# jbikker/tinybvh

Measured on AMD Instinct MI355X. Metric: MRays/s (primary + diffuse) on Bistro CWBVH, higher is better.
Workload: dtype f32; 1 GPU; procedural street (Bistro-exterior stand-in, 2.83M tris, seed 2); BVH8_CWBVH; per GPU per step 16777216 primary + 16777216 diffuse (depth 1-3) Intersect; scene_tris=2832120, layout=BVH8_CWBVH, scene_is_stand_in=True

## Files before the change

include/tinybvh_amd_debug.h:

```cpp
#ifndef TINYBVH_AMD_DEBUG_H_
#define TINYBVH_AMD_DEBUG_H_
#include "tinybvh_amd.h"
#ifdef __cplusplus
extern "C" {
#endif

int tbvh_debug_stats(tbvh_context* ctx, uint64_t out[8], int reset);

int tbvh_debug_set_flags(tbvh_context* ctx, uint32_t flags);

int tbvh_debug_coherent_schedule(tbvh_scene* scene, int anyhit, uint32_t out[4]);

int tbvh_debug_last_probe(tbvh_context* ctx, uint32_t out[3]);

int tbvh_debug_overlap_stats(tbvh_context* ctx, uint64_t out[2]);
int tbvh_debug_lane_script(const uint64_t* ops5, uint64_t n_ops, int32_t* out);

int tbvh_set_variant(tbvh_scene* scene, int variant);

int tbvh_debug_wide_copy_bvh2(int layout, const void* blob, uint64_t n_blob, const uint32_t* prim_idx, uint64_t n_idx, const void* verts16, uint64_t n_tris,
                              uint32_t max_leaf_tris, void* nodes32_out, uint64_t cap_nodes, uint64_t* n_nodes_out, void* recs_out, uint64_t cap_recs,
                              uint64_t* n_recs_out);

int tbvh_debug_set_sah_small_subtree(tbvh_context* ctx, uint32_t n);

int tbvh_debug_device_allocations(uint64_t out[2]);

struct tbvh_scenegraph;
int tbvh_debug_scenegraph_array(struct tbvh_scenegraph* g, int what, void** d_ptr);
int tbvh_debug_scenegraph_step(struct tbvh_scenegraph* g, int step, float dt);
struct tbvh_host_scenegraph;
int tbvh_debug_host_scenegraph_set_trs(struct tbvh_host_scenegraph* g, const float* trs10, uint64_t n_nodes);
int tbvh_debug_host_scenegraph_check_chains(struct tbvh_host_scenegraph* g, uint64_t* n_differ);

#ifdef __cplusplus
}
#endif
#endif
```

tinybvh_amd/_capi.py:

```python
from __future__ import annotations

import ctypes as C
import os

_HERE = os.path.dirname(os.path.abspath(__file__))
LIB_PATH = os.environ.get("TBVH_LIB_OVERRIDE") or os.path.join(_HERE, "libtinybvh_amd.so")

_u64, _u32, _vp, _i = C.c_uint64, C.c_uint32, C.c_void_p, C.c_int
_pp = C.POINTER(C.c_void_p)


class BuildParams(C.Structure):
    _fields_ = [("bins", _u32), ("max_leaf_tris", _u32), ("threads", _u32), ("flags", _u32)]


class Mesh(C.Structure):
    _fields_ = [("verts", C.c_void_p), ("n_verts", C.c_uint64), ("stride_bytes", C.c_uint32), ("on_device", C.c_uint32),
                ("indices", C.c_void_p), ("n_tris", C.c_uint64)]


class AlphaTexture(C.Structure):
    _fields_ = [("texels", C.c_void_p), ("width", C.c_uint32), ("height", C.c_uint32)]


class OmmSource(C.Structure):
    _fields_ = [("uv", C.c_void_p), ("n_uv", C.c_uint64), ("uv_stride_bytes", C.c_uint32), ("on_device", C.c_uint32), ("indices", C.c_void_p),
                ("n_tris", C.c_uint64), ("tri_texture", C.c_void_p), ("textures", C.POINTER(AlphaTexture)), ("n_textures", C.c_uint32)]


class SceneGraphDesc(C.Structure):
    _fields_ = [("flags", C.c_uint32), ("n_nodes", C.c_uint64), ("parent", C.c_void_p), ("visit_order", C.c_void_p), ("translation", C.c_void_p), ("rotation", C.c_void_p),
                ("scale", C.c_void_p), ("matrix", C.c_void_p), ("local_transform", C.c_void_p), ("n_weights", C.c_void_p), ("weights", C.c_void_p),
                ("n_samplers", C.c_uint64), ("sampler_interpolation", C.c_void_p), ("sampler_type", C.c_void_p), ("sampler_key_offset", C.c_void_p),
                ("sampler_value_offset", C.c_void_p), ("key_times", C.c_void_p), ("key_values", C.c_void_p), ("n_animations", C.c_uint64), ("n_channels", C.c_uint64),
                ("channel_animation", C.c_void_p), ("channel_sampler", C.c_void_p), ("channel_node", C.c_void_p), ("channel_target", C.c_void_p),
                ("n_instances", C.c_uint64), ("node_of_instance", C.c_void_p), ("n_skin_uses", C.c_uint64), ("skin_mesh_node", C.c_void_p),
                ("skin_joint_offset", C.c_void_p), ("skin_joint_node", C.c_void_p), ("skin_inverse_bind", C.c_void_p)]


class Camera(C.Structure):
    _fields_ = [("eye", C.c_float * 3), ("p1", C.c_float * 3), ("p2", C.c_float * 3), ("p3", C.c_float * 3),
                ("width", _u32), ("height", _u32), ("spp_x", _u32), ("spp_y", _u32)]


class WfParams(C.Structure):
    _fields_ = [("light_pos", C.c_float * 3), ("light_color", C.c_float * 3), ("sky_lo", C.c_float * 3), ("sky_hi", C.c_float * 3),
                ("eps", C.c_float), ("max_depth", _u32), ("seed", _u32), ("clear", _u32), ("light_size", C.c_float * 2), ("flags", _u32), ("sample_index", _u32)]


class WfStats(C.Structure):
    _fields_ = [("extend_rays", _u64 * 8), ("shadow_rays", _u64 * 8), ("frame_ms", C.c_float)]


SYMBOLS = {
    "tbvh_debug_wide_copy_bvh2": (_i, [_i, _vp, _u64, _vp, _u64, _vp, _u64, _u32, _vp, _u64, C.POINTER(_u64), _vp, _u64, C.POINTER(_u64)]),
    "tbvh_wavefront_create": (_i, [_vp, _u32, _u32, _pp]),
    "tbvh_wavefront_destroy": (None, [_vp]),
    "tbvh_wavefront_render": (_i, [_vp, _vp, _vp, C.POINTER(Camera), C.POINTER(WfParams), C.POINTER(WfStats)]),
    "tbvh_wavefront_read": (_i, [_vp, _vp]),
    "tbvh_wavefront_set_blas_vertices": (_i, [_vp, _vp, _u64]),
    "tbvh_wavefront_finalize": (_i, [_vp, C.c_float, _vp]),
    "tbvh_wavefront_set_blue_noise": (_i, [_vp, _vp, _u64]),
    "tbvh_abi_version": (_i, []),
    "tbvh_last_error": (C.c_char_p, []),
    "tbvh_device_count": (_i, []),
    "tbvh_init": (_i, [_i, _pp]),
    "tbvh_shutdown": (None, [_vp]),
    "tbvh_synchronize": (_i, [_vp]),
    "tbvh_set_stream": (_i, [_vp, _vp]),
    "tbvh_context_set_overlap": (_i, [_vp, _i]),
    "tbvh_debug_overlap_stats": (_i, [_vp, _vp]),
    "tbvh_debug_lane_script": (_i, [_vp, _u64, _vp]),
    "tbvh_set_timing": (_i, [_vp, _i]),
    "tbvh_upload_bvh_gpu": (_i, [_vp, _vp, _u64, _vp, _u64, _vp, _u64, _pp]),
    "tbvh_upload_bvh4_gpu": (_i, [_vp, _vp, _u64, _pp]),
    "tbvh_upload_cwbvh": (_i, [_vp, _vp, _u64, _vp, _u64, _pp]),
    "tbvh_upload_tlas": (_i, [_vp, _vp, _u64, _vp, _u64, _vp, _u64, _pp, _u64, _pp]),
    "tbvh_update_tlas": (_i, [_vp, _vp, _u64, _vp, _u64, _vp, _u64]),
    "tbvh_update_bvh_gpu": (_i, [_vp, _vp, _u64, _vp, _u64, _vp, _u64]),
    "tbvh_update_bvh4_gpu": (_i, [_vp, _vp, _u64]),
    "tbvh_update_cwbvh": (_i, [_vp, _vp, _u64, _vp, _u64]),
    "tbvh_rebuild_tlas_device": (_i, [_vp, _vp, _i, _vp, _u64]),
    "tbvh_refit": (_i, [_vp, _vp, _u64, _i]),
    "tbvh_set_opacity_micromaps": (_i, [_vp, _vp, _u32, _u64, _i]),
    "tbvh_scene_download": (_i, [_vp, _i, _vp, _u64, _vp]),
    "tbvh_build_device": (_i, [_vp, _vp, _u64, _i, _i, _u32, _vp]),
    "tbvh_build_device_ploc": (_i, [_vp, _vp, _u64, _i, _i, _u32, _vp]),
    "tbvh_build_device_sah": (_i, [_vp, _vp, _u64, _i, _i, _u32, _vp]),
    "tbvh_build_bvh2_sah_device": (_i, [_vp, C.POINTER(Mesh), _u32, _vp, _u64, _vp, _u64, _i, C.POINTER(_u64)]),
    "tbvh_host_build_bvh2_sah": (_i, [C.POINTER(Mesh), _u32, _vp, _u64, _vp, _u64, C.POINTER(_u64)]),
    "tbvh_convert_bvh2_device": (_i, [_vp, _vp, _u64, _vp, _u64, _vp, _u64, _i, _i, _vp]),
    "tbvh_tlas_download": (_i, [_vp, _vp, _u64, _vp, _u64, _vp, _u64, _vp]),
    "tbvh_free_scene": (None, [_vp]),
    "tbvh_scene_layout": (_i, [_vp]),
    "tbvh_scene_device_bytes": (_u64, [_vp]),
    "tbvh_intersect": (_i, [_vp, _vp, _u64, _u32]),
    "tbvh_occluded": (_i, [_vp, _vp, _u64, _u32, _vp]),
    "tbvh_intersect_sharded": (_i, [_vp, _u32, _vp, _u64, _u32]),
    "tbvh_occluded_sharded": (_i, [_vp, _u32, _vp, _u64, _u32, _vp]),
    "tbvh_intersect_sharded_device": (_i, [_vp, _u32, _vp, _vp, _i, C.c_float, _vp, _vp]),
    "tbvh_occluded_sharded_device": (_i, [_vp, _u32, _vp, _vp, _vp, _vp, _vp]),
    "tbvh_wavefront_set_band": (_i, [_vp, _u32, _u32]),
    "tbvh_wavefront_render_sharded": (_i, [_vp, _vp, _vp, _u32, C.POINTER(Camera), _vp, _vp, _vp]),
    "tbvh_wavefront_read_sharded": (_i, [_vp, _u32, _vp]),
    "tbvh_shard_range": (None, [_u64, _u32, _u32, C.POINTER(_u64), C.POINTER(_u64)]),
    "tbvh_intersect_device": (_i, [_vp, _vp, _u64]),
    "tbvh_occluded_device": (_i, [_vp, _vp, _u64, _vp]),
    "tbvh_intersect_device_fresh": (_i, [_vp, _vp, _u64, C.c_float]),
    "tbvh_reset_hits_device": (_i, [_vp, _vp, _u64, C.c_float]),
    "tbvh_time_last_ms": (C.c_float, [_vp]),
    "tbvh_debug_coherent_schedule": (C.c_int, [_vp, C.c_int, C.POINTER(C.c_uint32)]),
    "tbvh_time_history": (C.c_int, [_vp, C.POINTER(C.c_float), C.c_uint32, C.POINTER(C.c_uint32)]),
    "tbvh_measure_copy_bandwidth": (_i, [_vp, _u64, _u32, C.POINTER(C.c_double)]),
    "tbvh_measure_read_bandwidth": (_i, [_vp, _u64, _u32, C.POINTER(C.c_double)]),
    "tbvh_measure_valu_issue": (_i, [_vp, _u32, C.POINTER(C.c_double)]),
    "tbvh_measure_link_bandwidth": (_i, [_vp, _u64, _u32, C.POINTER(C.c_double), C.POINTER(C.c_double)]),
    "tbvh_scene_get_schedule_hint": (_i, [_vp, _vp]),
    "tbvh_scene_set_schedule_hint": (_i, [_vp, _vp]),
    "tbvh_pinned_malloc": (_i, [_vp, _u64, _pp]),
    "tbvh_pinned_free": (_i, [_vp, _vp]),
    "tbvh_set_variant": (_i, [_vp, _i]),
    "tbvh_debug_stats": (_i, [_vp, _vp, _i]),
    "tbvh_debug_last_probe": (_i, [_vp, _vp]),
    "tbvh_debug_set_flags": (_i, [_vp, _u32]),
    "tbvh_debug_set_sah_small_subtree": (_i, [_vp, _u32]),
    "tbvh_debug_device_allocations": (_i, [C.POINTER(_u64)]),
    "tbvh_cwbvh_set_hybrid": (_i, [_vp, C.c_int64]),
    "tbvh_bin_rays_device": (_i, [_vp, _vp, _vp, _u64, C.POINTER(C.c_float), _u32, _u32, _vp]),
    "tbvh_generate_primary_device": (_i, [_vp, C.POINTER(Camera), _vp, _u64, _u64]),
    "tbvh_generate_bounce_device": (_i, [_vp, _vp, _vp, _vp, _u64, _u32]),
    "tbvh_generate_shadow_device": (_i, [_vp, _vp, _vp, _u64, C.POINTER(C.c_float), C.c_float]),
    "tbvh_device_malloc": (_i, [_vp, _u64, _pp]),
    "tbvh_device_free": (_i, [_vp, _vp]),
    "tbvh_copy_to_device": (_i, [_vp, _vp, _vp, _u64]),
    "tbvh_copy_from_device": (_i, [_vp, _vp, _vp, _u64]),
    "tbvh_host_build": (_i, [_vp, _u64, _i, C.POINTER(BuildParams), _pp]),
    "tbvh_host_build_tlas": (_i, [_vp, _u64, _vp, _u64, _pp]),
    "tbvh_host_free": (None, [_vp]),
    "tbvh_cwbvh_file_write": (_i, [C.c_char_p, _vp, _u64, _vp, _u64, _u64, _vp]),
    "tbvh_cwbvh_file_read": (_i, [C.c_char_p, _u64, _pp, C.POINTER(_u64)]),
    "tbvh_host_layout": (_i, [_vp]),
    "tbvh_host_blob": (_vp, [_vp, _i]),
    "tbvh_host_blob_count": (_u64, [_vp, _i]),
    "tbvh_upload_host": (_i, [_vp, _vp, _vp, _u64, _pp]),
    "tbvh_upload_bvh_double": (_i, [_vp, _vp, _u64, _vp, _u64, _vp, _u64, _pp]),
    "tbvh_upload_tlas_double": (_i, [_vp, _vp, _u64, _vp, _u64, _vp, _u64, _pp, _u64, _pp]),
    "tbvh_intersect_ex_device": (_i, [_vp, _vp, _u64]),
    "tbvh_occluded_ex_device": (_i, [_vp, _vp, _u64, _vp]),
    "tbvh_intersect_ex": (_i, [_vp, _vp, _u64]),
    "tbvh_occluded_ex": (_i, [_vp, _vp, _u64, _vp]),
    "tbvh_host_build_double": (_i, [_vp, _u64, _pp]),
    "tbvh_host_build_tlas_double": (_i, [_vp, _u64, _vp, _u64, _pp]),
    "tbvh_rebuild_tlas_double_device": (_i, [_vp, _vp, _i]),
    "tbvh_update_tlas_double": (_i, [_vp, _vp, _u64, _vp, _u64, _vp, _u64]),
    "tbvh_tlas_double_download": (_i, [_vp, _vp, _u64, _vp, _u64, _vp, _u64, _vp]),
# ... 109 lines not shown
```

tinybvh_amd/csrc/capi_context.hip:

```cpp
#include "capi_internal.h"

using namespace tbvh;
using namespace tbvh_capi;

namespace {
thread_local char g_err[512] = "";
}

namespace tbvh_capi {
int fail(int code, const char* fmt, ...) {
    va_list ap;
    va_start(ap, fmt);
    vsnprintf(g_err, sizeof g_err, fmt, ap);
    va_end(ap);
    return code;
}

int joinLanes(tbvh_context* c) {
    if (c->lane1Dirty) {
        HIP_TRY(hipStreamWaitEvent(c->stream, c->lane1Last, 0));
        c->lane1Dirty = false;
        c->laneJoins++;
    }
    c->book.joined();
    c->lane0Touched = true;
    c->chain++;
    if (!c->chain) c->chain = 1;
    return 0;
}
int setDevice(tbvh_context* c) {
    HIP_TRY(hipSetDevice(c->device));
    return joinLanes(c);
}
hipError_t timedBegin(tbvh_context* c, hipStream_t lane) {
    if (c->skipTiming) return hipSuccess;
    const uint32_t slot = (uint32_t)(c->evSeq % tbvh_context::kTimeRing);
    for (int k = 0; k < 2; k++)
        if (!c->evRing[slot][k]) { const hipError_t e = hipEventCreate(&c->evRing[slot][k]); if (e != hipSuccess) return e; }
    c->evDone[slot] = false;
    c->evChain[slot] = 0;
    c->ev0 = c->evRing[slot][0]; c->ev1 = c->evRing[slot][1];
    c->evSeq++;
    return hipEventRecord(c->ev0, lane ? lane : c->stream);
}
hipError_t timedEnd(tbvh_context* c, hipStream_t lane) {
    if (c->skipTiming) return hipSuccess;
    const hipError_t e = hipEventRecord(c->ev1, lane ? lane : c->stream);
    if (e == hipSuccess && c->evSeq) { c->evDone[(c->evSeq - 1) % tbvh_context::kTimeRing] = true; c->timed = true; }
    return e;
}
float timedMs(tbvh_context* c, uint64_t seq) {
    constexpr uint64_t R = tbvh_context::kTimeRing;
    const uint32_t slot = (uint32_t)(seq % R);
    float own = -1.0f;
    if (hipEventElapsedTime(&own, c->evRing[slot][0], c->evRing[slot][1]) != hipSuccess) { (void)hipGetLastError(); return -1.0f; }
    const uint32_t chain = c->evChain[slot];
    if (!chain) return own;
    constexpr uint64_t kReach = 2 * LaneBook::kMaxInFlight;
    const uint64_t oldest = c->evSeq > R ? c->evSeq - R : 0;
    const uint64_t lo = seq > oldest + kReach ? seq - kReach : oldest, hi = seq + kReach < c->evSeq ? seq + kReach + 1 : c->evSeq;
    float from = 0.f;
    for (uint64_t j = lo; j < hi; j++) {
        const uint32_t sj = (uint32_t)(j % R);
        if (j == seq || c->evChain[sj] != chain || !c->evDone[sj]) continue;
        float endJ = 0.f;
        if (hipEventSynchronize(c->evRing[sj][1]) != hipSuccess || hipEventElapsedTime(&endJ, c->evRing[slot][0], c->evRing[sj][1]) != hipSuccess) { (void)hipGetLastError(); continue; }
        const bool before = endJ < own || (endJ == own && j < seq);
        if (before && endJ > from) from = endJ;
    }
    return own - from;
}
}

extern "C" {

int tbvh_abi_version(void) { return TBVH_ABI_VERSION; }
const char* tbvh_last_error(void) { return g_err; }

int tbvh_device_count(void) {
    int n = 0;
    hipError_t e = hipGetDeviceCount(&n);
    if (e != hipSuccess) { fail(TBVH_E_HIP, "hipGetDeviceCount: %s", hipGetErrorString(e)); return e == hipErrorNoDevice ? 0 : TBVH_E_HIP; }
    return n;
// ... 56 lines not shown
    if (c->lane1.stream) hipStreamSynchronize(c->lane1.stream);
    if (c->ownStream) hipStreamSynchronize(c->ownStream);
    c->lane1Dirty = false;
    for (;;) {
        tbvh_scene* t = nullptr;
        for (tbvh_scene* s : c->scenes) if (s->isTlas) { t = s; break; }
        if (!t) break;
        tbvh_free_scene(t);
    }
    while (!c->scenes.empty()) tbvh_free_scene(c->scenes.back());
    freePosesOf(c);
    freeGraphsOf(c);
    freeShadingsOf(c);
    freeOmmStagingOf(c);
    for (const tbvh_context::PinnedRange& r : c->pinned) hipHostFree(r.host);
    c->pinned.clear();
    delete c->pipe;
    for (auto& pair : c->evRing) for (hipEvent_t ev : pair) if (ev) hipEventDestroy(ev);
    if (c->evBase) hipEventDestroy(c->evBase);
    if (c->lane1.stream) hipStreamDestroy(c->lane1.stream);
    if (c->ownStream) hipStreamDestroy(c->ownStream);
    delete c;
}

int tbvh_debug_device_allocations(uint64_t out[2]) {
    if (!out) return fail(TBVH_E_INVALID, "tbvh_debug_device_allocations: null argument");
    out[0] = g_devBufLive.load(); out[1] = g_devBufBytes.load();
    return 0;
}

int tbvh_synchronize(tbvh_context* c) {
    if (!c) return fail(TBVH_E_INVALID, "null context");
    TBVH_ENTER(c);
    HIP_TRY(hipStreamSynchronize(c->stream));
    return 0;
}

int tbvh_set_stream(tbvh_context* c, void* s) {
    if (!c) return fail(TBVH_E_INVALID, "null context");
    TBVH_ENTER(c);
    c->stream = s ? (hipStream_t)s : c->ownStream;
    return 0;
}

int tbvh_context_set_overlap(tbvh_context* c, int enabled) {
    if (!c) return fail(TBVH_E_INVALID, "tbvh_context_set_overlap: null context");
    TBVH_ENTER(c);
    c->overlap = enabled != 0;
    return 0;
}

int tbvh_debug_lane_script(const uint64_t* ops5, uint64_t nOps, int32_t* out) {
    if ((!ops5 || !out) && nOps) return fail(TBVH_E_INVALID, "tbvh_debug_lane_script: null argument");
    LaneBook book;
    std::vector<uint8_t> done(nOps, 0);
    bool allowLane1 = true;
    auto prune = [&] { book.prune([&](int, uint32_t slot) { return done[slot] != 0; }); };
    for (uint64_t i = 0; i < nOps; i++) {
        const uint64_t* op = ops5 + i * 5;
        out[i] = 0;
        switch (op[0]) {
        case 0: {
            LaneFootprint fp;
            fp.rays.lo = (uintptr_t)op[1]; fp.rays.hi = (uintptr_t)op[2]; fp.occ.lo = (uintptr_t)op[3]; fp.occ.hi = (uintptr_t)op[4];
            prune();
            const LaneChoice ch = book.decide(fp, allowLane1);
            if (ch.join) book.joined();
            book.add(ch.lane, fp, (uint32_t)i);
            out[i] = ch.lane + (ch.join ? 2 : 0);
            break;
        }
        case 1:
            if (op[1] >= nOps) return fail(TBVH_E_INVALID, "tbvh_debug_lane_script: row %llu finishes a row beyond the script", (unsigned long long)i);
            done[op[1]] = 1;
            break;
        case 2: allowLane1 = op[1] != 0; break;
        case 3: prune(); out[i] = book.count[0] + 256 * book.count[1]; break;
        default: return fail(TBVH_E_INVALID, "tbvh_debug_lane_script: row %llu has no such operation", (unsigned long long)i);
        }
    }
    return 0;
}

int tbvh_debug_overlap_stats(tbvh_context* c, uint64_t out[2]) {
    if (!c || !out) return fail(TBVH_E_INVALID, "tbvh_debug_overlap_stats: null argument");
    TBVH_LOCK(c);
    out[0] = c->lane1Launches; out[1] = c->laneJoins;
    return 0;
}

float tbvh_time_last_ms(tbvh_context* c) {
    if (!c) return -1.0f;
    TBVH_LOCK(c);
    if (!c->timed) return -1.0f;
    if (c->hostQuerySeq == c->evSeq && c->hostQueryMs >= 0.f) return c->hostQueryMs;
    hipSetDevice(c->device);
    if (hipEventSynchronize(c->ev1) != hipSuccess) return -1.0f;
    if (c->evSeq && c->ev1 == c->evRing[(c->evSeq - 1) % tbvh_context::kTimeRing][1]) return timedMs(c, c->evSeq - 1);
    float ms = -1.0f;
    if (hipEventElapsedTime(&ms, c->ev0, c->ev1) != hipSuccess) return -1.0f;
    return ms;
}

int tbvh_time_history(tbvh_context* c, float* ms, uint32_t cap, uint32_t* count) {
    if (!c || !count || (!ms && cap)) return fail(TBVH_E_INVALID, "tbvh_time_history: null argument");
    *count = 0;
    TBVH_ENTER(c);
    uint64_t n = c->evSeq < tbvh_context::kTimeRing ? c->evSeq : tbvh_context::kTimeRing;
    if (n > cap) n = cap;
    for (uint64_t i = 0; i < n; i++) {
        const uint32_t slot = (uint32_t)((c->evSeq - n + i) % tbvh_context::kTimeRing);
        float t = -1.0f;
        if (c->evDone[slot]) {
            HIP_TRY(hipEventSynchronize(c->evRing[slot][1]));
            t = timedMs(c, c->evSeq - n + i);
            if (t < 0.f && !c->evChain[slot]) HIP_TRY(hipEventElapsedTime(&t, c->evRing[slot][0], c->evRing[slot][1]));
        }
        ms[i] = t;
    }
    *count = (uint32_t)n;
    return 0;
}

int tbvh_debug_stats(tbvh_context* c, uint64_t out[8], int reset) {
    if (!c || !out) return fail(TBVH_E_INVALID, "tbvh_debug_stats: null argument");
    TBVH_ENTER(c);
    HIP_TRY(hipStreamSynchronize(c->stream));
    HIP_TRY(hipMemcpy(out, c->counter + 8, 64, hipMemcpyDeviceToHost));
    if (reset) HIP_TRY(hipMemset(c->counter + 8, 0, 64));
    return 0;
}

int tbvh_set_timing(tbvh_context* c, int enabled) {
    if (!c) return fail(TBVH_E_INVALID, "tbvh_set_timing: null context");
    TBVH_LOCK(c);
    c->skipTiming = enabled == 0;
    return 0;
}

int tbvh_debug_set_flags(tbvh_context* c, uint32_t flags) {
    if (!c) return fail(TBVH_E_INVALID, "tbvh_debug_set_flags: null context");
    TBVH_LOCK(c);
    c->expFlags = flags;
    return 0;
}

int tbvh_debug_last_probe(tbvh_context* c, uint32_t out[3]) {
    if (!c || !out) return fail(TBVH_E_INVALID, "tbvh_debug_last_probe: null argument");
    TBVH_ENTER(c);
    out[0] = out[1] = out[2] = 0;
    if (!c->lastProbed) return 0;
    HIP_TRY(hipStreamSynchronize(c->stream));
    const uint32_t* pool = c->lastProbedLane ? c->lane1.pool.get() : c->pool.get();
    const int last = (c->lastProbedLane ? c->lane1.poolCur : c->poolCur) ^ 1;
    HIP_TRY(hipMemcpy(out, pool + (size_t)last * ((size_t)(kPoolParts + 1) * kPoolCounterStride) + (size_t)kPoolParts * kPoolCounterStride, 8, hipMemcpyDeviceToHost));
    out[2] = (out[1] != 0 && out[0] * 10u >= out[1] * 6u) ? 2u : 1u;
    return 0;
}


int tbvh_device_malloc(tbvh_context* c, uint64_t bytes, void** out) {
    if (!c || !out) return fail(TBVH_E_INVALID, "tbvh_device_malloc: null argument");
    TBVH_ENTER(c);
    hipError_t e = hipMalloc(out, bytes ? bytes : 16);
    if (e != hipSuccess) return fail(TBVH_E_NOMEM, "hipMalloc(%llu): %s", (unsigned long long)bytes, hipGetErrorString(e));
    return 0;
// ... 108 lines not shown
```

tinybvh_amd/csrc/cwbvh_packet.h:

```cpp
#pragma once
#include "device_common.h"
#include "cwbvh_node.h"

namespace tbvh {

constexpr int kPacketWG = 64;

__device__ __forceinline__ uint32_t sgpr(uint32_t v) { return (uint32_t)__builtin_amdgcn_readfirstlane((int)v); }

template <bool MIXED>
__device__ __forceinline__ uint32_t pk_test_children(const float (*planes)[8], float ax, float ay, float az, float ox, float oy, float oz, float tcull,
                                                     uint32_t m0, uint32_t m1, uint32_t oct0) {
    const uint32_t lane = threadIdx.x;
    const uint32_t metaL = ((lane & 4u) ? m1 : m0) >> (8u * (lane & 3u)) & 255u;
    const bool innerL = (metaL & 0x18u) == 0x18u;
    const uint32_t placedL = (metaL >> 5) << ((innerL ? (metaL ^ oct0) : metaL) & 31u);
    const uint32_t nonEmpty = (uint32_t)wave_ballot(lane < 8u && metaL != 0u);
    uint32_t hitmask = 0;
    float4 pa = *(const float4*)&planes[0][0];
    float2 pb = *(const float2*)&planes[0][4];
#pragma unroll
    for (int c = 0; c < 8; c++) {
        const float4 qa = pa; const float2 qb = pb;
        if (c < 7) { pa = *(const float4*)&planes[c + 1][0]; pb = *(const float2*)&planes[c + 1][4]; }
        if (!((nonEmpty >> c) & 1u)) continue;
        float tnx = __builtin_fmaf(qa.x, ax, ox), tny = __builtin_fmaf(qa.y, ay, oy), tnz = __builtin_fmaf(qa.z, az, oz);
        float tfx = __builtin_fmaf(qa.w, ax, ox), tfy = __builtin_fmaf(qb.x, ay, oy), tfz = __builtin_fmaf(qb.y, az, oz);
        if (MIXED) {
            const float a0 = __builtin_fminf(tnx, tfx), a1 = __builtin_fmaxf(tnx, tfx), b0 = __builtin_fminf(tny, tfy), b1 = __builtin_fmaxf(tny, tfy);
            const float c0 = __builtin_fminf(tnz, tfz), c1 = __builtin_fmaxf(tnz, tfz);
            tnx = a0; tfx = a1; tny = b0; tfy = b1; tnz = c0; tfz = c1;
        }
        const float cmin = __builtin_fmaxf(cw_fmax3(tnx, tny, tnz), 0.0f);
        const float cmax = __builtin_fminf(cw_fmin3(tfx, tfy, tfz), tcull);
        const uint32_t placed = (uint32_t)__builtin_amdgcn_readlane((int)placedL, c);
        hitmask |= wave_ballot(cmin <= cmax) != 0ull ? placed : 0u;
    }
    return hitmask;
}

}
```

tinybvh_amd/csrc/kernels_cwbvh_packet.hip:

```cpp
#include "device_common.h"
#include "ray_pool.h"
#include "kernels.h"
#include "cwbvh_node.h"
#include "cwbvh_probe.h"
#include "cwbvh_packet.h"

namespace tbvh {

namespace {

constexpr int WG = 64;

template <bool ANYHIT, bool HAS_OMM>
__global__ __launch_bounds__(WG, 8) void k_cwbvh_packet(const float4* __restrict__ nodes, const float4* __restrict__ tris, QueryArgs q, uint32_t* __restrict__ status) {
    __shared__ float planes[8][8];
    const uint64_t nRaysTotal = q.nRaysDev ? *q.nRaysDev : q.nRays;
    RayPool<64> pool;
    pool.init(q.poolParts, q.counterNext);
    if (q.probe) {
        uint32_t agree, pairs;
        coherence_sample(q.rays, nRaysTotal, q.fresh != 0u, q.freshTmax, agree, pairs);
        if (blockIdx.x == 0 && threadIdx.x == 0) { q.probe[0] = agree; q.probe[1] = pairs; }
        if (!((pairs != 0 && agree * 10u >= pairs * 6u) || (q.flags & 16u) != 0)) return;
    }
    uint2* const spill = (uint2*)q.spill + (size_t)blockIdx.x * WG;
    const size_t spillRow = (size_t)gridDim.x * WG;
    const uint32_t spillCap = q.spillStride * (uint32_t)WG;
    bool overflow = false;
    const uint32_t lane = threadIdx.x;

    for (;;) {
        uint64_t ri = 0;
        const bool have = pool.acquire(true, q.counter, nRaysTotal, ri);
        if (wave_ballot(have) == 0) break;
        float3 O = make_float3(0, 0, 0), D = make_float3(0, 0, 1), rD = make_float3(1e30f, 1e30f, 1);
        float4 hit = make_float4(0, 0, 0, 0);
        if (have) {
            const RayRec* rp = q.rays + ri;
            O = xyz(rp->O); D = xyz(rp->D); rD = xyz(rp->rD);
            hit = q.fresh ? make_float4(q.freshTmax, 0.f, 0.f, 0.f) : rp->hit;
        }
        bool found = false;
        bool on = have;
        const uint32_t oct = 7u - ((rD.x < 0 ? 4u : 0u) | (rD.y < 0 ? 2u : 0u) | (rD.z < 0 ? 1u : 0u));
        const unsigned long long haveMask = wave_ballot(have);
        const uint32_t first = (uint32_t)__builtin_ctzll(haveMask);
        const uint32_t oct0 = (uint32_t)__builtin_amdgcn_readlane((int)oct, (int)first);
        const bool mixed = wave_ballot(have && oct != oct0) != 0;
        const bool negX0 = ((7u - oct0) & 4u) != 0, negY0 = ((7u - oct0) & 2u) != 0, negZ0 = ((7u - oct0) & 1u) != 0;
        const uint32_t p = lane >> 3, axis = p % 3u, isHi = p / 3u;
        const bool negA = axis == 0 ? negX0 : axis == 1 ? negY0 : negZ0;
        const uint32_t dstPlane = axis + 3u * (isHi ^ (negA ? 1u : 0u));
        float* const myPlane = &planes[lane & 7u][lane < 48u ? dstPlane : 6u + ((lane >> 3) & 1u)];

        uint32_t sp = 0;
        uint32_t ngx = 0, ngy = 0x80000000u;
        uint32_t stkx = 0, stky = 0;
        auto pick = [&](uint32_t& ci) -> bool {
            if (!(ngy > 0x00FFFFFFu)) {
                if (sp == 0) return false;
                sp--;
                if (sp < 64u) { ngx = (uint32_t)__builtin_amdgcn_readlane((int)stkx, (int)sp); ngy = (uint32_t)__builtin_amdgcn_readlane((int)stky, (int)sp); }
                else { const uint32_t j_ = sp - 64u; const uint2 e = spill[(j_ & 63u) + (size_t)(j_ >> 6) * spillRow]; ngx = sgpr(e.x); ngy = sgpr(e.y); }
            }
            const uint32_t imaskWord = ngy;
            const uint32_t bit = 31u - (uint32_t)__builtin_clz(ngy);
            ngy &= ~(1u << bit);
            if (ngy > 0x00FFFFFFu) {
                if (sp < 64u) { const bool mine = lane == sp; stkx = mine ? ngx : stkx; stky = mine ? ngy : stky; }
                else {
                    const uint32_t j_ = sp - 64u;
                    if (j_ < spillCap) { if (lane == 0) spill[(j_ & 63u) + (size_t)(j_ >> 6) * spillRow] = make_uint2(ngx, ngy); }
                    else { overflow = true; sp--; }
                }
                sp++;
            }
            const uint32_t slot = (bit - 24u) ^ oct0;
            ci = sgpr(ngx + (uint32_t)__popc(imaskWord & ~(0xFFFFFFFFu << slot)));
            return true;
        };
        uint32_t ci = 0;
        bool more = pick(ci);
        float4 n0 = make_float4(0, 0, 0, 0), n1 = n0;
        uint32_t qb = 0;
        auto fetch = [&](uint32_t c_) {
            const float4* np = nodes + (size_t)c_ * 5u;
            n0 = np[0]; n1 = np[1];
            qb = ((const uint8_t*)(np + 2))[lane < 48u ? lane : 47u];
        };
        if (more) fetch(ci);
        while (more) {
            __builtin_amdgcn_wave_barrier();
            *myPlane = (float)qb;
            __builtin_amdgcn_wave_barrier();
            const uint32_t ew = sgpr(as_u32(n0.w));
            const float ax = ldexpf(rD.x, (int)(int8_t)(ew)), ay = ldexpf(rD.y, (int)(int8_t)(ew >> 8)), az = ldexpf(rD.z, (int)(int8_t)(ew >> 16));
            const float ox = (n0.x - O.x) * rD.x, oy = (n0.y - O.y) * rD.y, oz = (n0.z - O.z) * rD.z;
            const bool lives = ANYHIT ? (on && !found) : on;
            const float tcull = lives ? cull_bound(hit.x) : -1.0f;
            const uint32_t m0 = sgpr(as_u32(n1.z)), m1 = sgpr(as_u32(n1.w));
            const uint32_t hitmask = mixed ? pk_test_children<true>(planes, ax, ay, az, ox, oy, oz, tcull, m0, m1, oct0)
                                           : pk_test_children<false>(planes, ax, ay, az, ox, oy, oz, tcull, m0, m1, oct0);
            ngx = sgpr(as_u32(n1.x));
            ngy = (hitmask & 0xFF000000u) | (ew >> 24);
            uint32_t tgy = hitmask & 0x00FFFFFFu;
            const uint32_t tgx = sgpr(as_u32(n1.y));
            more = pick(ci);
            if (more) fetch(ci);
            while (tgy != 0u) {
                const uint32_t ti = 31u - (uint32_t)__builtin_clz(tgy);
                tgy &= ~(1u << ti);
                const float4* tp = tris + ((size_t)tgx + ti * 3u);
                const float4 e2 = tp[0], e1 = tp[1], v0 = tp[2];
                TriHit h;
                if ((ANYHIT ? (on && !found) : on) &&
                    tri_test(O, D, xyz(v0), xyz(e1), xyz(e2), hit.x, h, HAS_OMM ? q.omm : Omm{nullptr, 0}, as_u32(v0.w)) &&
                    (ANYHIT || hit_wins(h.t, as_u32(v0.w), found, hit))) {
                    found = true;
                    if (!ANYHIT) hit = make_float4(h.t, h.u, h.v, v0.w);
                }
            }
            if (ANYHIT && wave_ballot(on && !found) == 0ull) break;
        }
        if (have) {
            if (ANYHIT) q.occluded[ri] = found ? 1 : 0;
            else if (found || q.fresh) q.rays[ri].hit = hit;
        }
    }
    if (overflow) atomicOr(status, 1u);
}

}

void launch_cwbvh_packet(bool anyhit, const float4* nodes, const float4* tris, const QueryArgs& q, uint32_t* status, uint32_t blocks, hipStream_t s) {
    if (anyhit) {
        if (q.omm.map) hipLaunchKernelGGL((k_cwbvh_packet<true, true>), dim3(blocks), dim3(WG), 0, s, nodes, tris, q, status);
        else hipLaunchKernelGGL((k_cwbvh_packet<true, false>), dim3(blocks), dim3(WG), 0, s, nodes, tris, q, status);
    } else {
        if (q.omm.map) hipLaunchKernelGGL((k_cwbvh_packet<false, true>), dim3(blocks), dim3(WG), 0, s, nodes, tris, q, status);
        else hipLaunchKernelGGL((k_cwbvh_packet<false, false>), dim3(blocks), dim3(WG), 0, s, nodes, tris, q, status);
    }
}

}
```

Baseline: 5166 MRays/s.

## Add conservative packet-interval culling of CWBVH children before per-lane exact tests

For coherent, non-anyhit packets whose rays share one octant and are all finite, the kernel computes wave-wide min/max of origins and inverse directions plus the maximum cull distance. Each node's child boxes are then tested once against this interval bound, and only surviving children get the exact per-lane ballot test. The aim is to skip per-child FMA work and ballots for children no ray can hit. In exchange it adds wave reductions at packet start and after every hit update, more shared memory, and extra per-node plane math. It also adds a host debug entry point that reproduces the cull logic.

```diff
diff --git a/include/tinybvh_amd_debug.h b/include/tinybvh_amd_debug.h
--- a/include/tinybvh_amd_debug.h
+++ b/include/tinybvh_amd_debug.h
@@ -15,6 +15,9 @@
 
 int tbvh_debug_overlap_stats(tbvh_context* ctx, uint64_t out[2]);
 int tbvh_debug_lane_script(const uint64_t* ops5, uint64_t n_ops, int32_t* out);
+
+int tbvh_debug_packet_cull(const void* nodes80, uint64_t n_nodes, const void* rays64, uint64_t have_mask, const float* tcull64, uint8_t* maybe_out,
+                           uint8_t* exact_out, uint32_t* chunk_flags);
 
 int tbvh_set_variant(tbvh_scene* scene, int variant);
 
diff --git a/tinybvh_amd/_capi.py b/tinybvh_amd/_capi.py
--- a/tinybvh_amd/_capi.py
+++ b/tinybvh_amd/_capi.py
@@ -71,6 +71,7 @@
     "tbvh_context_set_overlap": (_i, [_vp, _i]),
     "tbvh_debug_overlap_stats": (_i, [_vp, _vp]),
     "tbvh_debug_lane_script": (_i, [_vp, _u64, _vp]),
+    "tbvh_debug_packet_cull": (_i, [_vp, _u64, _vp, _u64, _vp, _vp, _vp, _vp]),
     "tbvh_set_timing": (_i, [_vp, _i]),
     "tbvh_upload_bvh_gpu": (_i, [_vp, _vp, _u64, _vp, _u64, _vp, _u64, _pp]),
     "tbvh_upload_bvh4_gpu": (_i, [_vp, _vp, _u64, _pp]),
diff --git a/tinybvh_amd/csrc/capi_context.hip b/tinybvh_amd/csrc/capi_context.hip
--- a/tinybvh_amd/csrc/capi_context.hip
+++ b/tinybvh_amd/csrc/capi_context.hip
@@ -1,4 +1,5 @@
 #include "capi_internal.h"
+#include "packet_cull.h"
 
 using namespace tbvh;
 using namespace tbvh_capi;
@@ -221,6 +222,75 @@
     return 0;
 }
 
+int tbvh_debug_packet_cull(const void* nodes80, uint64_t nNodes, const void* rays64, uint64_t haveMask, const float* tcull64, uint8_t* maybeOut, uint8_t* exactOut,
+                           uint32_t* chunkFlags) {
+    if (!rays64 || !tcull64 || haveMask == 0 || (nNodes && (!nodes80 || !maybeOut || !exactOut)))
+        return fail(TBVH_E_INVALID, "tbvh_debug_packet_cull: null argument or no lane holds a ray");
+    using namespace tbvh;
+    float O[64][3], rD[64][3];
+    uint32_t oct[64];
+    for (int l = 0; l < 64; l++) {
+        const float* r = (const float*)((const uint8_t*)rays64 + 64 * l);
+        for (int a = 0; a < 3; a++) { O[l][a] = r[a]; rD[l][a] = r[8 + a]; }
+        oct[l] = 7u - ((rD[l][0] < 0 ? 4u : 0u) | (rD[l][1] < 0 ? 2u : 0u) | (rD[l][2] < 0 ? 1u : 0u));
+    }
+    const int first = __builtin_ctzll(haveMask);
+    const uint32_t oct0 = oct[first];
+    const bool neg0[3] = {((7u - oct0) & 4u) != 0, ((7u - oct0) & 2u) != 0, ((7u - oct0) & 1u) != 0};
+    bool mixed = false, raysFinite = true;
+    float Olo[3], Ohi[3], rlo[3], rhi[3], TC = -1.0f;
+    for (int a = 0; a < 3; a++) { Olo[a] = Ohi[a] = O[first][a]; rlo[a] = rhi[a] = rD[first][a]; }
+    for (int l = 0; l < 64; l++) {
+        if (!((haveMask >> l) & 1u)) continue;
+        mixed |= oct[l] != oct0;
+        for (int a = 0; a < 3; a++) {
+            raysFinite &= pkc_finite(O[l][a]) && pkc_finite(rD[l][a]);
+            Olo[a] = __builtin_fminf(Olo[a], O[l][a]); Ohi[a] = __builtin_fmaxf(Ohi[a], O[l][a]);
+            rlo[a] = __builtin_fminf(rlo[a], rD[l][a]); rhi[a] = __builtin_fmaxf(rhi[a], rD[l][a]);
+        }
+        TC = __builtin_fmaxf(TC, pk_cull_tc(tcull64[l]));
+    }
+    const bool useCull = !mixed && raysFinite;
+    if (chunkFlags) *chunkFlags = (mixed ? 1u : 0u) | (raysFinite ? 0u : 2u);
+    for (uint64_t n = 0; n < nNodes; n++) {
+        const uint8_t* node = (const uint8_t*)nodes80 + 80 * n;
+        float n0[3];
+        uint32_t ew;
+        memcpy(n0, node, 12); memcpy(&ew, node + 12, 4);
+        const int e[3] = {(int)(int8_t)ew, (int)(int8_t)(ew >> 8), (int)(int8_t)(ew >> 16)};
+        const uint8_t* meta = node + 24;
+        const uint8_t* qbytes = node + 32;
+        float planes[8][6], bounds[8][6];
+        bool allFinite = true;
+        for (uint32_t L = 0; L < 48; L++) {
+            const uint32_t p = L >> 3, axis = p % 3u, isHi = p / 3u, dstPlane = axis + 3u * (isHi ^ (neg0[axis] ? 1u : 0u));
+            const float qf = (float)qbytes[L];
+            planes[L & 7u][dstPlane] = qf;
+            bool fin;
+            bounds[L & 7u][dstPlane] = pk_cull_plane(dstPlane >= 3u, qf, n0[axis], e[axis], Olo[axis], Ohi[axis], rlo[axis], rhi[axis], fin);
+            allFinite &= fin;
+        }
+        float ax[64][3], ox[64][3];
+        for (int l = 0; l < 64; l++)
+            for (int a = 0; a < 3; a++) { ax[l][a] = ldexpf(rD[l][a], e[a]); ox[l][a] = (n0[a] - O[l][a]) * rD[l][a]; }
+        uint32_t maybe = 0, exact = 0;
+        for (uint32_t c = 0; c < 8; c++) {
+            if (meta[c] == 0) continue;
+            const float* b = bounds[c];
+            if (!useCull || pk_cull_pass(b[0], b[1], b[2], b[3], b[4], b[5], TC, allFinite)) maybe |= 1u << c;
+            const float* q = planes[c];
+            for (int l = 0; l < 64 && !((exact >> c) & 1u); l++) {
+                if (!((haveMask >> l) & 1u)) continue;
+                const bool in = mixed ? pk_child_exact<true>(q[0], q[1], q[2], q[3], q[4], q[5], ax[l][0], ax[l][1], ax[l][2], ox[l][0], ox[l][1], ox[l][2], tcull64[l])
+                                      : pk_child_exact<false>(q[0], q[1], q[2], q[3], q[4], q[5], ax[l][0], ax[l][1], ax[l][2], ox[l][0], ox[l][1], ox[l][2], tcull64[l]);
+                if (in) exact |= 1u << c;
+            }
+        }
+        maybeOut[n] = (uint8_t)maybe; exactOut[n] = (uint8_t)exact;
+    }
+    return 0;
+}
+
 int tbvh_debug_overlap_stats(tbvh_context* c, uint64_t out[2]) {
     if (!c || !out) return fail(TBVH_E_INVALID, "tbvh_debug_overlap_stats: null argument");
     TBVH_LOCK(c);
diff --git a/tinybvh_amd/csrc/cwbvh_packet.h b/tinybvh_amd/csrc/cwbvh_packet.h
--- a/tinybvh_amd/csrc/cwbvh_packet.h
+++ b/tinybvh_amd/csrc/cwbvh_packet.h
@@ -1,6 +1,7 @@
 #pragma once
 #include "device_common.h"
 #include "cwbvh_node.h"
+#include "packet_cull.h"
 
 namespace tbvh {
 
@@ -8,14 +9,20 @@
 
 __device__ __forceinline__ uint32_t sgpr(uint32_t v) { return (uint32_t)__builtin_amdgcn_readfirstlane((int)v); }
 
-template <bool MIXED>
-__device__ __forceinline__ uint32_t pk_test_children(const float (*planes)[8], float ax, float ay, float az, float ox, float oy, float oz, float tcull,
-                                                     uint32_t m0, uint32_t m1, uint32_t oct0) {
+struct PkMeta { uint32_t placedL, nonEmpty; };
+__device__ __forceinline__ PkMeta pk_meta(uint32_t m0, uint32_t m1, uint32_t oct0) {
     const uint32_t lane = threadIdx.x;
     const uint32_t metaL = ((lane & 4u) ? m1 : m0) >> (8u * (lane & 3u)) & 255u;
     const bool innerL = (metaL & 0x18u) == 0x18u;
-    const uint32_t placedL = (metaL >> 5) << ((innerL ? (metaL ^ oct0) : metaL) & 31u);
-    const uint32_t nonEmpty = (uint32_t)wave_ballot(lane < 8u && metaL != 0u);
+    PkMeta m;
+    m.placedL = (metaL >> 5) << ((innerL ? (metaL ^ oct0) : metaL) & 31u);
+    m.nonEmpty = (uint32_t)wave_ballot(metaL != 0u) & 0xFFu;
+    return m;
+}
+
+template <bool MIXED>
+__device__ __forceinline__ uint32_t pk_test_children_of(const float (*planes)[8], float ax, float ay, float az, float ox, float oy, float oz, float tcull,
+                                                        uint32_t placedL, uint32_t todo) {
     uint32_t hitmask = 0;
     float4 pa = *(const float4*)&planes[0][0];
     float2 pb = *(const float2*)&planes[0][4];
@@ -23,20 +30,43 @@
     for (int c = 0; c < 8; c++) {
         const float4 qa = pa; const float2 qb = pb;
         if (c < 7) { pa = *(const float4*)&planes[c + 1][0]; pb = *(const float2*)&planes[c + 1][4]; }
-        if (!((nonEmpty >> c) & 1u)) continue;
-        float tnx = __builtin_fmaf(qa.x, ax, ox), tny = __builtin_fmaf(qa.y, ay, oy), tnz = __builtin_fmaf(qa.z, az, oz);
-        float tfx = __builtin_fmaf(qa.w, ax, ox), tfy = __builtin_fmaf(qb.x, ay, oy), tfz = __builtin_fmaf(qb.y, az, oz);
-        if (MIXED) {
-            const float a0 = __builtin_fminf(tnx, tfx), a1 = __builtin_fmaxf(tnx, tfx), b0 = __builtin_fminf(tny, tfy), b1 = __builtin_fmaxf(tny, tfy);
-            const float c0 = __builtin_fminf(tnz, tfz), c1 = __builtin_fmaxf(tnz, tfz);
-            tnx = a0; tfx = a1; tny = b0; tfy = b1; tnz = c0; tfz = c1;
-        }
-        const float cmin = __builtin_fmaxf(cw_fmax3(tnx, tny, tnz), 0.0f);
-        const float cmax = __builtin_fminf(cw_fmin3(tfx, tfy, tfz), tcull);
+        if (!((todo >> c) & 1u)) continue;
         const uint32_t placed = (uint32_t)__builtin_amdgcn_readlane((int)placedL, c);
-        hitmask |= wave_ballot(cmin <= cmax) != 0ull ? placed : 0u;
+        hitmask |= wave_ballot(pk_child_exact<MIXED>(qa.x, qa.y, qa.z, qa.w, qb.x, qb.y, ax, ay, az, ox, oy, oz, tcull)) != 0ull ? placed : 0u;
     }
     return hitmask;
 }
 
+template <bool MIXED>
+__device__ __forceinline__ uint32_t pk_test_children(const float (*planes)[8], float ax, float ay, float az, float ox, float oy, float oz, float tcull,
+                                                     uint32_t m0, uint32_t m1, uint32_t oct0) {
+    const PkMeta m = pk_meta(m0, m1, oct0);
+    return pk_test_children_of<MIXED>(planes, ax, ay, az, ox, oy, oz, tcull, m.placedL, m.nonEmpty);
 }
+
+__device__ __forceinline__ uint32_t pk_test_survivors(const float (*planes)[8], float ax, float ay, float az, float ox, float oy, float oz, float tcull,
+                                                      uint32_t placedL, uint32_t todo) {
+    uint32_t hitmask = 0;
+    while (todo != 0u) {
+        const uint32_t c = (uint32_t)__builtin_ctz(todo);
+        todo &= todo - 1u;
+        const float4 qa = *(const float4*)&planes[c][0];
+        const float2 qb = *(const float2*)&planes[c][4];
+        const uint32_t placed = (uint32_t)__builtin_amdgcn_readlane((int)placedL, (int)c);
+        hitmask |= wave_ballot(pk_child_exact<false>(qa.x, qa.y, qa.z, qa.w, qb.x, qb.y, ax, ay, az, ox, oy, oz, tcull)) != 0ull ? placed : 0u;
+    }
+    return hitmask;
+}
+
+template <bool MAX>
+__device__ __forceinline__ float pk_wave_reduce(float v) {
+#define TBVH_PK_ROR(n) { const float o_ = __int_as_float(__builtin_amdgcn_update_dpp(0, __float_as_int(v), 0x120 + (n), 0xF, 0xF, false)); \
+                         v = MAX ? __builtin_fmaxf(v, o_) : __builtin_fminf(v, o_); }
+    TBVH_PK_ROR(1) TBVH_PK_ROR(2) TBVH_PK_ROR(4) TBVH_PK_ROR(8)
+#undef TBVH_PK_ROR
+    const float r0 = __int_as_float(__builtin_amdgcn_readlane(__float_as_int(v), 0)), r1 = __int_as_float(__builtin_amdgcn_readlane(__float_as_int(v), 16));
+    const float r2 = __int_as_float(__builtin_amdgcn_readlane(__float_as_int(v), 32)), r3 = __int_as_float(__builtin_amdgcn_readlane(__float_as_int(v), 48));
+    return MAX ? __builtin_fmaxf(__builtin_fmaxf(r0, r1), __builtin_fmaxf(r2, r3)) : __builtin_fminf(__builtin_fminf(r0, r1), __builtin_fminf(r2, r3));
+}
+
+}
diff --git a/tinybvh_amd/csrc/kernels_cwbvh_packet.hip b/tinybvh_amd/csrc/kernels_cwbvh_packet.hip
--- a/tinybvh_amd/csrc/kernels_cwbvh_packet.hip
+++ b/tinybvh_amd/csrc/kernels_cwbvh_packet.hip
@@ -13,7 +13,7 @@
 
 template <bool ANYHIT, bool HAS_OMM>
 __global__ __launch_bounds__(WG, 8) void k_cwbvh_packet(const float4* __restrict__ nodes, const float4* __restrict__ tris, QueryArgs q, uint32_t* __restrict__ status) {
-    __shared__ float planes[8][8];
+    __shared__ float planes[16][8];
     const uint64_t nRaysTotal = q.nRaysDev ? *q.nRaysDev : q.nRays;
     RayPool<64> pool;
     pool.init(q.poolParts, q.counterNext);
@@ -53,6 +53,25 @@
         const uint32_t dstPlane = axis + 3u * (isHi ^ (negA ? 1u : 0u));
         float* const myPlane = &planes[lane & 7u][lane < 48u ? dstPlane : 6u + ((lane >> 3) & 1u)];
 
+        const bool farL = dstPlane >= 3u;
+        const bool rayFinite = pkc_finite(O.x) && pkc_finite(O.y) && pkc_finite(O.z) && pkc_finite(rD.x) && pkc_finite(rD.y) && pkc_finite(rD.z);
+        const bool useCull = !ANYHIT && !mixed && wave_ballot(have && !rayFinite) == 0ull;
+        float cOlo = 0, cOhi = 0, crlo = 0, crhi = 0, TC = 0;
+        auto refreshTC = [&]() {
+            TC = as_f32(sgpr(as_u32(pk_wave_reduce<true>(pk_cull_tc(on ? cull_bound(hit.x) : -1.0f)))));
+        };
+        if (useCull) {
+            auto first_or = [&](float v) { return have ? v : __int_as_float(__builtin_amdgcn_readlane(__float_as_int(v), (int)first)); };
+            const float3 Of = make_float3(first_or(O.x), first_or(O.y), first_or(O.z)), rf = make_float3(first_or(rD.x), first_or(rD.y), first_or(rD.z));
+            const float oxl = pk_wave_reduce<false>(Of.x), oyl = pk_wave_reduce<false>(Of.y), ozl = pk_wave_reduce<false>(Of.z);
+            const float oxh = pk_wave_reduce<true>(Of.x), oyh = pk_wave_reduce<true>(Of.y), ozh = pk_wave_reduce<true>(Of.z);
+            const float rxl = pk_wave_reduce<false>(rf.x), ryl = pk_wave_reduce<false>(rf.y), rzl = pk_wave_reduce<false>(rf.z);
+            const float rxh = pk_wave_reduce<true>(rf.x), ryh = pk_wave_reduce<true>(rf.y), rzh = pk_wave_reduce<true>(rf.z);
+            cOlo = axis == 0 ? oxl : axis == 1 ? oyl : ozl; cOhi = axis == 0 ? oxh : axis == 1 ? oyh : ozh;
+            crlo = axis == 0 ? rxl : axis == 1 ? ryl : rzl; crhi = axis == 0 ? rxh : axis == 1 ? ryh : rzh;
+            refreshTC();
+        }
+
         uint32_t sp = 0;
         uint32_t ngx = 0, ngy = 0x80000000u;
         uint32_t stkx = 0, stky = 0;
@@ -91,22 +110,42 @@
         if (more) fetch(ci);
         while (more) {
             __builtin_amdgcn_wave_barrier();
-            *myPlane = (float)qb;
-            __builtin_amdgcn_wave_barrier();
+            const float qf = (float)qb;
+            *myPlane = qf;
             const uint32_t ew = sgpr(as_u32(n0.w));
-            const float ax = ldexpf(rD.x, (int)(int8_t)(ew)), ay = ldexpf(rD.y, (int)(int8_t)(ew >> 8)), az = ldexpf(rD.z, (int)(int8_t)(ew >> 16));
-            const float ox = (n0.x - O.x) * rD.x, oy = (n0.y - O.y) * rD.y, oz = (n0.z - O.z) * rD.z;
-            const bool lives = ANYHIT ? (on && !found) : on;
-            const float tcull = lives ? cull_bound(hit.x) : -1.0f;
             const uint32_t m0 = sgpr(as_u32(n1.z)), m1 = sgpr(as_u32(n1.w));
-            const uint32_t hitmask = mixed ? pk_test_children<true>(planes, ax, ay, az, ox, oy, oz, tcull, m0, m1, oct0)
-                                           : pk_test_children<false>(planes, ax, ay, az, ox, oy, oz, tcull, m0, m1, oct0);
+            const PkMeta meta = pk_meta(m0, m1, oct0);
+            uint32_t todo = meta.nonEmpty;
+            if (useCull) {
+                bool fin;
+                const float n0a = axis == 0 ? n0.x : axis == 1 ? n0.y : n0.z;
+                const float bound = pk_cull_plane(farL, qf, n0a, (int)(int8_t)(ew >> (8u * axis)), cOlo, cOhi, crlo, crhi, fin);
+                myPlane[64] = bound;
+                const bool allFinite = (wave_ballot(!fin) & 0x0000FFFFFFFFFFFFull) == 0ull;
+                __builtin_amdgcn_wave_barrier();
+                const float4 ba = *(const float4*)&planes[8u + (lane & 7u)][0];
+                const float2 bb = *(const float2*)&planes[8u + (lane & 7u)][4];
+                const uint32_t passMask = (uint32_t)wave_ballot(pk_cull_pass(ba.x, ba.y, ba.z, ba.w, bb.x, bb.y, TC, true));
+                if (allFinite) todo &= passMask;
+            } else __builtin_amdgcn_wave_barrier();
+            uint32_t hitmask = 0;
+            if (todo != 0u) {
+                const float ax = ldexpf(rD.x, (int)(int8_t)(ew)), ay = ldexpf(rD.y, (int)(int8_t)(ew >> 8)), az = ldexpf(rD.z, (int)(int8_t)(ew >> 16));
+                const float ox = (n0.x - O.x) * rD.x, oy = (n0.y - O.y) * rD.y, oz = (n0.z - O.z) * rD.z;
+                const bool lives = ANYHIT ? (on && !found) : on;
+                const float tcull = lives ? cull_bound(hit.x) : -1.0f;
+                if (mixed) hitmask = pk_test_children_of<true>(planes, ax, ay, az, ox, oy, oz, tcull, meta.placedL, todo);
+                else if (!useCull) hitmask = pk_test_children_of<false>(planes, ax, ay, az, ox, oy, oz, tcull, meta.placedL, todo);
+                else hitmask = pk_test_survivors(planes, ax, ay, az, ox, oy, oz, tcull, meta.placedL, todo);
+            }
             ngx = sgpr(as_u32(n1.x));
             ngy = (hitmask & 0xFF000000u) | (ew >> 24);
             uint32_t tgy = hitmask & 0x00FFFFFFu;
             const uint32_t tgx = sgpr(as_u32(n1.y));
             more = pick(ci);
             if (more) fetch(ci);
+            bool changed = false;
+            const bool hadTris = tgy != 0u;
             while (tgy != 0u) {
                 const uint32_t ti = 31u - (uint32_t)__builtin_clz(tgy);
                 tgy &= ~(1u << ti);
@@ -117,9 +156,11 @@
                     tri_test(O, D, xyz(v0), xyz(e1), xyz(e2), hit.x, h, HAS_OMM ? q.omm : Omm{nullptr, 0}, as_u32(v0.w)) &&
                     (ANYHIT || hit_wins(h.t, as_u32(v0.w), found, hit))) {
                     found = true;
+                    changed = true;
                     if (!ANYHIT) hit = make_float4(h.t, h.u, h.v, v0.w);
                 }
             }
+            if (useCull && hadTris && wave_ballot(changed) != 0ull) refreshTC();
             if (ANYHIT && wave_ballot(on && !found) == 0ull) break;
         }
         if (have) {
diff --git a/tinybvh_amd/csrc/packet_cull.h b/tinybvh_amd/csrc/packet_cull.h
--- /dev/null
+++ b/tinybvh_amd/csrc/packet_cull.h
@@ -0,0 +1,50 @@
+#pragma once
+#include <math.h>
+#include <stdint.h>
+
+#if defined(__HIPCC__)
+#define PKC_HD __host__ __device__ __forceinline__
+#else
+#define PKC_HD inline
+#endif
+
+namespace tbvh {
+
+PKC_HD float pkc_min3(float a, float b, float c) { return __builtin_fminf(__builtin_fminf(a, b), c); }
+PKC_HD float pkc_max3(float a, float b, float c) { return __builtin_fmaxf(__builtin_fmaxf(a, b), c); }
+PKC_HD bool pkc_finite(float x) { return __builtin_fabsf(x) <= 3.402823466e38f; }
+
+template <bool MIXED>
+PKC_HD bool pk_child_exact(float qnx, float qny, float qnz, float qfx, float qfy, float qfz, float ax, float ay, float az, float ox, float oy, float oz,
+                           float tcull) {
+    float tnx = __builtin_fmaf(qnx, ax, ox), tny = __builtin_fmaf(qny, ay, oy), tnz = __builtin_fmaf(qnz, az, oz);
+    float tfx = __builtin_fmaf(qfx, ax, ox), tfy = __builtin_fmaf(qfy, ay, oy), tfz = __builtin_fmaf(qfz, az, oz);
+    if (MIXED) {
+        const float a0 = __builtin_fminf(tnx, tfx), a1 = __builtin_fmaxf(tnx, tfx), b0 = __builtin_fminf(tny, tfy), b1 = __builtin_fmaxf(tny, tfy);
+        const float c0 = __builtin_fminf(tnz, tfz), c1 = __builtin_fmaxf(tnz, tfz);
+        tnx = a0; tfx = a1; tny = b0; tfy = b1; tnz = c0; tfz = c1;
+    }
+    const float cmin = __builtin_fmaxf(pkc_max3(tnx, tny, tnz), 0.0f);
+    const float cmax = __builtin_fminf(pkc_min3(tfx, tfy, tfz), tcull);
+    return cmin <= cmax;
+}
+
+PKC_HD float pk_cull_plane(bool isFar, float q, float n0a, int e, float Olo, float Ohi, float rlo, float rhi, bool& finite) {
+    const float A = ldexpf(isFar ? rhi : rlo, e);
+    const float dlo = n0a - Ohi, dhi = n0a - Olo;
+    const float p0 = dlo * rlo, p1 = dlo * rhi, p2 = dhi * rlo, p3 = dhi * rhi;
+    const float oxLo = __builtin_fminf(pkc_min3(p0, p1, p2), p3), oxHi = __builtin_fmaxf(pkc_max3(p0, p1, p2), p3);
+    const float bound = __builtin_fmaf(q, A, isFar ? oxHi : oxLo);
+    finite = pkc_finite((p0 + p1) + (p2 + p3)) && pkc_finite(bound);
+    return bound;
+}
+
+PKC_HD bool pk_cull_pass(float tnx, float tny, float tnz, float tfx, float tfy, float tfz, float TC, bool allFinite) {
+    const float lb = __builtin_fmaxf(pkc_max3(tnx, tny, tnz), 0.0f);
+    const float ub = __builtin_fminf(pkc_min3(tfx, tfy, tfz), TC);
+    return !allFinite || lb <= ub;
+}
+
+PKC_HD float pk_cull_tc(float tcull) { return tcull == tcull ? tcull : __builtin_inff(); }
+
+}
```

Result: faster. 5256 MRays/s (median of 6 runs) (+1.8%).
